# OPPO-Mente-Lab/X2I

Hardware: AMD Instinct MI355X
Metric: images/sec, FLUX-schnell 1024x1024 4-step (projector + denoise loop), whole job (higher is better)
Workload: dtype bf16; 1 GPU; BASELINE configs[1]: qwen3b conditioning (C=37,H=2048,S_txt=512) -> projector -> shuttle-3/FLUX-schnell DiT 1024x1024, 4 steps; batch_per_gpu=4, global_batch=4, parallelism=batch-sharded x1, graph=True

## Files before the change

### x2i_amd/csrc/c_api.hip

```cpp
#include <stdarg.h>
#include <stdio.h>

#include "x2i_common.h"
#include "x2i_kernels.h"

static thread_local char g_err[512] = "";

int x2i_set_error(int code, const char* fmt, ...) {
  va_list ap;
  va_start(ap, fmt);
  vsnprintf(g_err, sizeof(g_err), fmt, ap);
  va_end(ap);
  return code;
}

int x2i_check_launch(const char* what) {
  hipError_t e = hipGetLastError();
  if (e != hipSuccess) return x2i_set_error(X2I_ERR_HIP, "%s: launch failed: %s", what, hipGetErrorString(e));
  return X2I_OK;
}

#include <stdlib.h>
#include <string.h>

// ... 7 lines not shown
  return v && *v ? atoi(v) : dflt;
}
X2IOptions make_options() {
  X2IOptions o;
  o.gemm_tile = env_int("X2I_GEMM_TILE", 0);
  o.gemm_min256 = env_int("X2I_GEMM_MIN256", 128);
  o.gemm_gm = env_int("X2I_GEMM_GM", 0);
  o.gemm_split_tail = env_int("X2I_GEMM_NOSPLIT", 0) ? 0 : 1;
  o.gemm_w4 = env_int("X2I_GEMM_W4", 1);
  o.gemm_persist = env_int("X2I_GEMM_PERSIST", 1);
  o.gemm_fp8_persist = env_int("X2I_GEMM_FP8_PERSIST", 1);
  o.gemm_fx = env_int("X2I_GEMM_FX", 2);
  o.gemm_fx_nk = env_int("X2I_GEMM_FX_NK", 96);
  o.gemm_streamk = env_int("X2I_GEMM_STREAMK", 1);
  o.gemm_pair = env_int("X2I_GEMM_PAIR", 1);
  o.train_rows_wg = env_int("X2I_TRAIN_ROWS_WG", 1);
  o.attn_bwd_overlap = env_int("X2I_ATTN_BWD_OVERLAP", 1);
  o.conv256 = env_int("X2I_CONV256", 1);
  o.conv_w4 = env_int("X2I_CONV_W4", 1);
  o.conv_korder = env_int("X2I_CONV_KORDER", 1);
  o.attn_variant = env_int("X2I_ATTN_VARIANT", 0);
  o.attn_w16 = env_int("X2I_ATTN_W16", 1);
  o.attn_streamk = env_int("X2I_ATTN_STREAMK", 1);
  o.conv5_variant = env_int("X2I_CONV5_VARIANT", 0);
  o.fp8 = env_int("X2I_FP8", 0);
  o.last_gemm_tile = -1;
  o.attn_ablate = env_int("X2I_ATTN_ABLATE", 0);
  return o;
}
std::mutex g_smem_mu;
std::set<std::pair<const void*, int>> g_smem_done;
}

X2IOptions& x2i_options() {
  static X2IOptions o = make_options();
  return o;
}

int x2i_ensure_dynamic_smem(const void* kernel, int bytes) {
  int dev = 0;
  hipGetDevice(&dev);
// ... 28 lines not shown
                        need, (long long)a->workspace_bytes);
    return false;
  }
  *flags = (unsigned*)a->workspace;
  *slabs = (float*)((char*)a->workspace + 4096);
  return true;
}

extern "C" {

int x2i_abi_version(void) { return X2I_ABI_VERSION; }

static long long* opt_slot(X2IOptions& o, const char* name, int** as_int) {
  *as_int = nullptr;
#define X2I_OPT_INT(N_) if (!strcmp(name, #N_)) { *as_int = &o.N_; return nullptr; }
  X2I_OPT_INT(gemm_tile) X2I_OPT_INT(gemm_gm) X2I_OPT_INT(gemm_split_tail) X2I_OPT_INT(gemm_w4) X2I_OPT_INT(gemm_persist) X2I_OPT_INT(gemm_fp8_persist) X2I_OPT_INT(gemm_fx) X2I_OPT_INT(gemm_fx_nk) X2I_OPT_INT(gemm_streamk) X2I_OPT_INT(gemm_pair) X2I_OPT_INT(train_rows_wg) X2I_OPT_INT(attn_bwd_overlap) X2I_OPT_INT(attn_streamk) X2I_OPT_INT(conv256) X2I_OPT_INT(conv_w4) X2I_OPT_INT(conv_korder) X2I_OPT_INT(attn_variant) X2I_OPT_INT(attn_w16) X2I_OPT_INT(conv5_variant) X2I_OPT_INT(fp8) X2I_OPT_INT(last_gemm_tile)
#ifdef X2I_ABLATION
  X2I_OPT_INT(attn_ablate)
#endif
#undef X2I_OPT_INT
  if (!strcmp(name, "gemm_min256")) return &o.gemm_min256;
  return nullptr;
}

int x2i_set_option(const char* name, int64_t value) {
  if (!name) return x2i_set_error(X2I_ERR_ARG, "set_option: null name");
  int* ip;
  long long* lp = opt_slot(x2i_options(), name, &ip);
  if (ip) *ip = (int)value;
  else if (lp) *lp = (long long)value;
  else return x2i_set_error(X2I_ERR_ARG, "set_option: unknown option '%s'", name);
// ... 361 lines not shown
```

### x2i_amd/csrc/gemm.hip

```cpp
#include "gemm_device.h"

using namespace x2i_gemm;

namespace {

__global__ void gemm_naive_kernel(GemmP p, int batch) {
  const int n = blockIdx.x * blockDim.x + threadIdx.x;
  const long long mz = (long long)blockIdx.z * gridDim.y + blockIdx.y;
  const int z = (int)(mz / p.M), m = (int)(mz % p.M);
  if (n >= p.N || z >= batch) return;
  const bf16_t* a = p.A + (long long)z * p.a_bs + (long long)m * p.lda;
  const bf16_t* w = p.W + (long long)(z / p.wdiv) * p.w_bs + (long long)n * p.ldw;
  float acc = 0.f;
  for (int k = 0; k < p.K; ++k) acc = fmaf(bf16_to_f32(a[k]), bf16_to_f32(w[k]), acc);
  float v = acc + (p.bias ? bf16_to_f32(p.bias[(long long)(z / p.wdiv) * p.bias_gs + n]) : 0.f) + (p.bias2 ? p.bias2[(long long)z * p.bias2_bs + n] : 0.f);
  v = apply_act(v, p.act);
  if (p.res) {
    const float g = p.gate ? p.gate[(long long)z * p.gate_bs + n] : 1.f;
    v = fmaf(g, v, bf16_to_f32(p.res[(long long)z * p.r_bs + (long long)m * p.ldr + n]));
  }
  const long long coff = (long long)z * p.c_bs + (long long)m * p.ldc + n;
  if (p.out_f32) ((float*)p.C)[coff] = v;
  else ((bf16_t*)p.C)[coff] = f32_to_bf16(v);
  if (p.C2) p.C2[coff] = f32_to_bf16(apply_act(v, p.act2));
// ... 21 lines not shown
}

static void fill_gemm_p(const x2i_gemm_args* a, const x2i_qkv_desc* qd, GemmP& p) {
  p.A = (const bf16_t*)a->A; p.a_bs = a->a_batch_stride; p.lda = a->lda;
  p.W = (const bf16_t*)a->W; p.ldw = a->ldw; p.w_bs = a->w_batch_stride;
  p.wdiv = a->w_group > 0 ? a->w_group : 1; p.bias_gs = a->w_group > 0 ? a->N : 0;
  p.bias = (const bf16_t*)a->bias;
  p.C = a->C; p.c_bs = a->c_batch_stride; p.ldc = a->ldc;
  p.C2 = (bf16_t*)a->C2; p.act2 = a->act2;
  p.gate = a->gate; p.gate_bs = a->gate_batch_stride;
  p.res = (const bf16_t*)a->res; p.r_bs = a->res_batch_stride; p.ldr = a->ldr;
  p.bias2 = a->bias2; p.bias2_bs = a->bias2_batch_stride;
  p.M = a->M; p.N = a->N; p.K = a->K; p.act = a->act; p.out_f32 = a->out_f32;
  p.cH = p.cW = p.cCin = p.cOW = p.cKW = p.cStride = p.cPad = p.cUp = p.cPadW = p.cRowPitch = p.cKorder = 0; p.cMom = nullptr; p.cMomBlocks = 0;
  p.gm = 4;
  p.q_on = 0; p.q_H = p.q_Spad = p.q_tok_off = p.q_rpb = p.q_row0 = p.q_vperm = 0; p.q_eps = 0.f; p.q_qs = 1.f;
  p.q_nq = p.q_nk = nullptr; p.q_cos = p.q_sin = nullptr; p.q_Q = p.q_K = p.q_VT = nullptr;
  p.f_sa = p.f_sw = nullptr; p.f_sa_bs = 0; p.f_alpha = p.f_oinv = 1.f; p.f_out8 = 0;
  p.nbatch = 1; p.sk_on = 0; p.sk_slabs = nullptr; p.sk_flags = nullptr; p.fx_v0 = 0;
  if (qd) {
    p.q_on = 1; p.q_H = qd->H; p.q_Spad = qd->Spad; p.q_tok_off = qd->tok_off; p.q_rpb = qd->rows_per_sample; p.q_eps = qd->eps; p.q_qs = qd->q_scale == 0.f ? 1.f : qd->q_scale;
    p.q_nq = (const bf16_t*)qd->norm_q; p.q_nk = (const bf16_t*)qd->norm_k; p.q_cos = qd->cos; p.q_sin = qd->sin;
    p.q_Q = (bf16_t*)qd->Q; p.q_K = (bf16_t*)qd->K; p.q_VT = (bf16_t*)qd->VT; p.q_vperm = qd->vt_perm ? 1 : 0;
    p.ldc = a->N; p.c_bs = 0;
  }
}

static int pick_gm(int tn, int K) {
  const X2IOptions& opt = x2i_options();
  if (opt.gemm_gm > 0) return opt.gemm_gm;
  if (tn <= 16) return K >= 8192 ? 1 : 4;
  if (tn <= 64) return 6;
  return 2;
}

static bool persistent_ok(const x2i_gemm_args* a, const x2i_qkv_desc* qd) {
  const X2IOptions& opt = x2i_options();
  const bool res = a->res != nullptr;
  const bool fast = (a->K % BK == 0) && (a->lda % 8 == 0) && (a->ldw % 8 == 0) && (((uintptr_t)a->A & 15) == 0) && (((uintptr_t)a->W & 15) == 0) &&
                    ((a->a_batch_stride & 7) == 0) && ((long long)a->M * a->lda * 2 < 0x7f000000LL) && ((long long)a->N * a->ldw * 2 < 0x7f000000LL);
// ... 75 lines not shown
    if (rc) return rc;
    pp.p[0].fx_v0 = v0;
    for (int i = 0; i < 2; ++i) pp.p[i].sk_slabs = sk_slabs, pp.p[i].sk_flags = sk_flags;
    hipLaunchKernelGGL(kfx, dim3((unsigned)cus), dim3(256), SMEM2P_BYTES, stream, pp);
    opt.last_gemm_tile = 3256;
    return x2i_check_launch("gemm_pair (fx)");
  }
  if (rc) return rc;
  rc = x2i_ensure_dynamic_smem((const void*)kern, SMEM2P_BYTES);
  if (rc) return rc;
  const bool sk = streamk_for(a0, tiles, a0->K / BK, cus, &sk_slabs, &sk_flags, &rc);
  if (rc) return rc;
  pp.p[0].sk_on = sk ? 1 : 0; pp.p[0].sk_slabs = sk_slabs; pp.p[0].sk_flags = sk_flags;
  hipLaunchKernelGGL(kern, dim3((unsigned)(tiles < cus ? tiles : cus)), dim3(256), SMEM2P_BYTES, stream, pp);
  opt.last_gemm_tile = 2256;
  return x2i_check_launch("gemm_pair");
}

constexpr int MOM_SLABS = 64;
__device__ __forceinline__ f32x4_t mom_block_sum(const float* __restrict__ src, int r0, int r1, int n2, f32x4_t* red) {
  const int lanes = n2 >> 2, groups = 256 / lanes;
  const int l = threadIdx.x % lanes, g = threadIdx.x / lanes;
  f32x4_t a0 = {0.f, 0.f, 0.f, 0.f}, a1 = a0, a2 = a0, a3 = a0;
  if (g < groups) {
    const float* p = src + 4 * l;
    int rb = r0 + g;
    for (; rb + 3 * groups < r1; rb += 4 * groups) {
      a0 += *(const f32x4_t*)(p + (long long)rb * n2);
      a1 += *(const f32x4_t*)(p + (long long)(rb + groups) * n2);
      a2 += *(const f32x4_t*)(p + (long long)(rb + 2 * groups) * n2);
// ... 92 lines not shown
      if (rc) return rc;
    }
  }
  return x2i_check_launch("conv");
}

static int launch_gemm_impl(const x2i_gemm_args* a, const x2i_conv_desc* cd, const x2i_qkv_desc* qd, hipStream_t stream) {
  if (!a || !a->A || !a->W || (!a->C && !qd)) return x2i_set_error(X2I_ERR_ARG, "gemm: null pointer");
  const bool conv = cd != nullptr;
  if (a->M <= 0 || a->N <= 0 || a->K <= 0 || a->batch <= 0) return x2i_set_error(X2I_ERR_SHAPE, "gemm: bad shape M=%d N=%d K=%d batch=%d", a->M, a->N, a->K, a->batch);
  if (a->gate && !a->res) return x2i_set_error(X2I_ERR_ARG, "gemm: gate without residual");
  if (a->w_group < 0 || (a->w_group > 0 && (!a->w_batch_stride || qd || a->C2 || a->out_f32)))
    return x2i_set_error(X2I_ERR_ARG, "gemm: w_group=%d needs w_batch_stride != 0 and goes with the plain bf16 outputs only (no fused QKV / C2 / f32 output)", a->w_group);
  GemmP p;
  fill_gemm_p(a, qd, p);
  if (conv) {
    if (a->gate) return x2i_set_error(X2I_ERR_ARG, "conv: a gated residual is not part of the convolution epilogues (residual: plain add)");
    if (cd->Cin % 64 || cd->H <= 0 || cd->W <= 0 || cd->KH <= 0 || cd->KW <= 0 || cd->stride <= 0)
      return x2i_set_error(X2I_ERR_SHAPE, "conv: Cin must be a multiple of 64 (Cin=%d)", cd->Cin);
    if (cd->up < 0 || cd->up > 2) return x2i_set_error(X2I_ERR_ARG, "conv: up must be 0, 1 (x2 along H and W) or 2 (x2 along H only), got %d", cd->up);
    const int up_h = cd->up ? 1 : 0, up_w = cd->up == 1 ? 1 : 0, up = up_h | (up_w << 1);
    const int pad_w = cd->pad_w_p1 <= 0 ? cd->pad : cd->pad_w_p1 - 1;
    if (cd->KH * cd->KW > 32) return x2i_set_error(X2I_ERR_SHAPE, "conv: at most 32 filter taps (KH=%d KW=%d)", cd->KH, cd->KW);
    int OH = ((cd->H << up_h) + 2 * cd->pad - cd->KH) / cd->stride + 1;
    if (cd->out_h) {
      if (cd->out_h < 0 || (cd->out_h - 1) * cd->stride - cd->pad >= (cd->H << up_h)) return x2i_set_error(X2I_ERR_SHAPE, "conv: out_h=%d lies outside the input (H=%d pad=%d)", cd->out_h, cd->H, cd->pad);
      OH = cd->out_h;
    }
    int OW = ((cd->W << up_w) + 2 * pad_w - cd->KW) / cd->stride + 1;
    if (cd->out_w) {
// ... 128 lines not shown
    int tm_main = tm_all;
    if (!sk && force == 0 && !conv && full_rounds >= 1 && rem > 0 && (rem <= 96 || (rem <= 128 && full_rounds >= 8)) && opt.gemm_split_tail) {
      const long long tm_fit = (full_rounds * 256) / per_row;
      if (tm_fit >= 1 && tm_fit < tm_all) tm_main = (int)tm_fit;
    }
    GemmP pm = p;
    pm.gm = pick_gm(tn, a->K);
    pm.M = (tm_main < tm_all) ? tm_main * BM2 : a->M;
    pm.tilesM = tm_main; pm.tilesN = tn;
    pm.cMomBlocks = tm_main * 2;
    if (kernp) {
      rc = x2i_ensure_dynamic_smem((const void*)kernp, SMEM2P_BYTES);
      if (rc) return rc;
      pm.nbatch = a->batch;
      pm.sk_on = sk ? 1 : 0; pm.sk_slabs = sk_slabs; pm.sk_flags = sk_flags;
      const long long tiles = (long long)pm.tilesM * pm.tilesN * a->batch;
      hipLaunchKernelGGL(kernp, dim3((unsigned)(tiles < cus ? tiles : cus)), dim3(256), SMEM2P_BYTES, stream, pm);
    } else {
      hipLaunchKernelGGL(kern2, dim3(pm.tilesM * pm.tilesN, a->batch), dim3(threads2), SMEM2_BYTES, stream, pm);
    }
    opt.last_gemm_tile = 256 + (tm_main < tm_all ? 1000 : 0);
    if (tm_main < tm_all) {
      rc = x2i_ensure_dynamic_smem((const void*)kern, 4 * TILE_BYTES);
      if (rc) return rc;
      GemmP pt = p;
      const long long r0 = (long long)tm_main * BM2;
      pt.A = p.A + r0 * p.lda;
      pt.C = p.out_f32 ? (void*)((float*)p.C + r0 * p.ldc) : (void*)((bf16_t*)p.C + r0 * p.ldc);
      if (p.C2) pt.C2 = p.C2 + r0 * p.ldc;
      if (p.res) pt.res = p.res + r0 * p.ldr;
// ... 77 lines not shown
    return x2i_set_error(X2I_ERR_ALIGN, "gemm_fp8: N, ldc and c_batch_stride must be multiples of %d, C 16-byte aligned", nal + 1);
  if (out8 && (res || a->gate)) return x2i_set_error(X2I_ERR_ARG, "gemm_fp8: e4m3 output has no residual form");
  kern_t kern = pick_gemm256_fp8(a->act, res, out8);
  if (!kern) return x2i_set_error(X2I_ERR_ARG, "gemm_fp8: epilogue (act=%d%s%s) is not instantiated", a->act, res ? ", residual" : "", out8 ? ", e4m3 out" : "");
  GemmP p;
  p.A = (const bf16_t*)a->A; p.a_bs = a->a_batch_stride; p.lda = a->lda;
  p.W = (const bf16_t*)a->W; p.ldw = a->ldw; p.w_bs = 0; p.wdiv = 1; p.bias_gs = 0;
  p.bias = (const bf16_t*)a->bias;
  p.C = a->C; p.c_bs = a->c_batch_stride; p.ldc = a->ldc;
  p.C2 = nullptr; p.act2 = 0;
  p.gate = a->gate; p.gate_bs = a->gate_batch_stride;
  p.res = (const bf16_t*)a->res; p.r_bs = a->res_batch_stride; p.ldr = a->ldr;
  p.bias2 = a->bias2; p.bias2_bs = a->bias2_batch_stride;
  p.M = a->M; p.N = a->N; p.K = a->K; p.act = a->act; p.out_f32 = 0;
  p.cH = p.cW = p.cCin = p.cOW = p.cKW = p.cStride = p.cPad = p.cUp = p.cPadW = p.cRowPitch = p.cKorder = 0; p.cMom = nullptr; p.cMomBlocks = 0;
  p.q_on = 0; p.q_H = p.q_Spad = p.q_tok_off = p.q_rpb = p.q_row0 = p.q_vperm = 0; p.q_eps = 0.f; p.q_qs = 1.f;
  p.q_nq = p.q_nk = nullptr; p.q_cos = p.q_sin = nullptr; p.q_Q = p.q_K = p.q_VT = nullptr;
  if (qd) {
    p.q_on = 1; p.q_H = qd->H; p.q_Spad = qd->Spad; p.q_tok_off = qd->tok_off; p.q_rpb = qd->rows_per_sample; p.q_eps = qd->eps; p.q_qs = qd->q_scale == 0.f ? 1.f : qd->q_scale;
    p.q_nq = (const bf16_t*)qd->norm_q; p.q_nk = (const bf16_t*)qd->norm_k; p.q_cos = qd->cos; p.q_sin = qd->sin;
    p.q_Q = (bf16_t*)qd->Q; p.q_K = (bf16_t*)qd->K; p.q_VT = (bf16_t*)qd->VT; p.q_vperm = qd->vt_perm ? 1 : 0;
    p.ldc = a->N; p.c_bs = 0;
  }
  p.f_sa = f->a_scale; p.f_sa_bs = f->a_scale_batch_stride; p.f_sw = f->w_scale; p.f_alpha = f->alpha; p.f_oinv = f->out_inv_scale;
  p.f_out8 = out8 ? 1 : 0;
  p.nbatch = 1; p.sk_on = 0; p.sk_slabs = nullptr; p.sk_flags = nullptr; p.fx_v0 = 0;
#ifdef X2I_ABLATION
  p.act2 = a->act2;
#endif
  const int tm = (a->M + BM2 - 1) / BM2, tn = (a->N + BN2 - 1) / BN2;
  p.tilesM = tm; p.tilesN = tn;
// ... 36 lines not shown
```

### x2i_amd/csrc/gemm256p.hip

```cpp
#include <type_traits>
#include "gemm_device.h"
#include "gemm256p_epi.h"
#include "gemm256w_loop.inc"
#include "gemm256f8_loop.inc"

namespace x2i_gemm {
namespace {

__device__ __forceinline__ void epilogue_fx_slice(const GemmP& p, int z, int m_wave, int n_wave, int lane, char* stage, int slab0, int P, int j,
                                                  int tid) {
  typedef unsigned int u32x4 __attribute__((ext_vector_type(4)));
  typedef unsigned int u32x2 __attribute__((ext_vector_type(2)));
  const int mlane = lane & 15, ng = lane >> 4;
  const int srow = lane >> 3, sch = lane & 7;
  const float* b2 = p.bias2 ? p.bias2 + (long long)z * p.bias2_bs : nullptr;
#ifdef X2I_ABLATION
  if (p.act2 >= 80) b2 = nullptr;
#endif
  const float* gz = p.gate ? p.gate + (long long)z * p.gate_bs : nullptr;
  __amdgpu_buffer_rsrc_t r_rsrc = __builtin_amdgcn_make_buffer_rsrc((void*)(p.res + (long long)z * p.r_bs), 0, (uint32_t)(((long long)(p.M - 1) * p.ldr + p.N) * 2), 0x00020000);
  const uint32_t c_bytes = (uint32_t)(((long long)(p.M - 1) * p.ldc + p.N) * 2);
  __amdgpu_buffer_rsrc_t c_rsrc = __builtin_amdgcn_make_buffer_rsrc((void*)((bf16_t*)p.C + (long long)z * p.c_bs), 0, c_bytes, 0x00020000);
  const float* sbase = p.sk_slabs + (long long)slab0 * (SK_SLAB_BYTES / 4) + tid * 4;
  for (int q = j; q < 8; q += P) {
// ... 323 lines not shown
};

template <bool PAIR> using GemmArg = std::conditional_t<PAIR, GemmP2, GemmP>;
__device__ __forceinline__ const GemmP& prob(const GemmP& a, int) { return a; }
__device__ __forceinline__ const GemmP& first(const GemmP& a) { return a; }
__device__ __forceinline__ const GemmP& first(const GemmP2& a) { return a.p[0]; }
__device__ __forceinline__ const GemmP& second(const GemmP& a) { return a; }
__device__ __forceinline__ const GemmP& second(const GemmP2& a) { return a.p[1]; }
__device__ __forceinline__ GemmP prob(const GemmP2& a, int sel) {
  const GemmP &x = a.p[0], &y = a.p[1];
  GemmP q;
#define X2I_F(f) q.f = sel ? y.f : x.f;
  X2I_F(A) X2I_F(a_bs) X2I_F(lda) X2I_F(W) X2I_F(ldw) X2I_F(w_bs) X2I_F(bias) X2I_F(C) X2I_F(c_bs) X2I_F(ldc) X2I_F(C2) X2I_F(act2)
  X2I_F(gate) X2I_F(gate_bs) X2I_F(res) X2I_F(r_bs) X2I_F(ldr) X2I_F(bias2) X2I_F(bias2_bs) X2I_F(M) X2I_F(N) X2I_F(K) X2I_F(act)
  X2I_F(out_f32) X2I_F(tilesM) X2I_F(tilesN) X2I_F(cH) X2I_F(cW) X2I_F(cCin) X2I_F(cOW) X2I_F(cKW) X2I_F(cStride) X2I_F(cPad) X2I_F(cUp) X2I_F(cPadW) X2I_F(cRowPitch) X2I_F(cKorder) X2I_F(cMom) X2I_F(cMomBlocks)
  X2I_F(q_on) X2I_F(q_H) X2I_F(q_Spad) X2I_F(q_tok_off) X2I_F(q_rpb) X2I_F(q_row0) X2I_F(q_vperm) X2I_F(gm) X2I_F(q_eps) X2I_F(q_qs) X2I_F(q_nq) X2I_F(q_nk)
  X2I_F(q_cos) X2I_F(q_sin) X2I_F(q_Q) X2I_F(q_K) X2I_F(q_VT) X2I_F(f_sa) X2I_F(f_sa_bs) X2I_F(f_sw) X2I_F(f_alpha) X2I_F(f_oinv) X2I_F(f_out8)
  X2I_F(nbatch) X2I_F(sk_on) X2I_F(sk_slabs) X2I_F(sk_flags) X2I_F(fx_v0)
#undef X2I_F
  return q;
}

template <int ACT, bool RES, bool HASC2, bool QKV = false, bool PAIR = false, bool F8 = false, bool OUT8 = false, bool FX = false>
__global__ __launch_bounds__(256) void gemm256p_kernel(GemmArg<PAIR> pp) {
  constexpr int ES = F8 ? 1 : 2;
  constexpr int KT = F8 ? 128 : BK;
  extern __shared__ __attribute__((aligned(16))) char smem[];
  const GemmP& p = first(pp);
  const int tid = threadIdx.x;
  const int lane = tid & 63;
  const int wave = __builtin_amdgcn_readfirstlane(tid >> 6);
// ... 11 lines not shown
    const int v = vb - sel * TT0;
    z = v / T;
    int bid = v - z * T;
    const int qq = T >> 3, r = T & 7, xcd = bid & 7, idx = bid >> 3;
    bid = (xcd < r ? xcd * (qq + 1) : r * (qq + 1) + (xcd - r) * qq) + idx;
    const int GM = q.gm;
    const int per_group = GM * q.tilesN;
    const int group = bid / per_group;
    const int first_m = group * GM;
    const int gsize = min(q.tilesM - first_m, GM);
    m0 = (first_m + (bid % per_group) % gsize) * BM2;
    n0 = ((bid % per_group) / gsize) * BN2;
  };
  const int khl = lane >> 5, r8 = (lane >> 2) & 7, cphys = lane & 3;
  const int kby = khl * 64 + ((cphys ^ (3 * (wave & 1))) << 4);
  auto offsets = [&](int sel, int z, int m0, int n0, uint32_t (&va)[8], uint32_t (&vw)[8]) {
    const GemmP& q = prob(pp, sel);
#ifdef X2I_ABLATION
    if (p.act2 == 75) m0 = 0, n0 = 0;
    if (p.act2 == 76) m0 &= 1023, n0 &= 2047;
#endif
    const long long zoff = (long long)z * q.a_bs;
#pragma unroll
    for (int jj = 0; jj < 8; ++jj) {
      const int row = (jj * 4 + wave) * 8 + r8;
      va[jj] = (m0 + row < q.M) ? (uint32_t)((zoff + (long long)(m0 + row) * q.lda) * ES + kby) : 0x80000000u;
      vw[jj] = (n0 + row < q.N) ? (uint32_t)(((long long)(n0 + row) * q.ldw) * ES + kby) : 0x80000000u;
    }
  };
  auto uni = [](auto v) { return (decltype(v))__builtin_amdgcn_readfirstlane((int)v); };
  auto mk_rsrc = [&](const void* ptr, uint32_t bytes) {
    const unsigned long long a = (unsigned long long)(uintptr_t)ptr;
    const unsigned long long au = ((unsigned long long)(unsigned)uni((int)(a >> 32)) << 32) | (unsigned)uni((int)(a & 0xffffffffu));
    return __builtin_amdgcn_make_buffer_rsrc((void*)(uintptr_t)au, 0, (uint32_t)uni((int)bytes), 0x00020000);
  };
  auto a_rsrc_of = [&](int sel) {
    const GemmP& q = prob(pp, sel);
    return mk_rsrc(q.A, (uint32_t)(((long long)(q.nbatch - 1) * q.a_bs + (long long)(q.M - 1) * q.lda + q.K) * ES));
  };
  auto w_rsrc_of = [&](int sel) {
    const GemmP& q = prob(pp, sel);
    return mk_rsrc(q.W, (uint32_t)(((long long)(q.N - 1) * q.ldw + q.K) * ES));
  };
  int fx_sel = 0, fx_Tp = 0, fx_nbz = 0, fx_kind = 0, fx_cnt = 0, fx_t0 = 0, fx_tstep = 1, fx_k0 = 0, fx_len = 0, fx_npre = 0, fx_modeB = 0, fx_slab_base = 0, fx_part = 0;
  const int fx_x = w & 7;
  if constexpr (FX) {
    const int wi = w >> 3, Gx = G >> 3;
    const int v0 = p.fx_v0;
    fx_sel = PAIR ? min(max(wi - v0 + 1, 0), 1) : 0;
    const GemmP& q = prob(pp, fx_sel);
    const int li = wi - fx_sel * v0, v = fx_sel ? Gx - v0 : v0;
    fx_Tp = q.tilesM * q.tilesN;
    fx_nbz = q.nbatch;
    fx_slab_base = fx_sel * (first(pp).tilesM * first(pp).tilesN);
    const int Tx = fx_Tp >> 3;
    if (v < 2 * Tx) {
      fx_modeB = 1;
// ... 124 lines not shown
    if (tid == 0) {
      for (int q = 0; q < P; ++q) fx_spin(fx_flag(buf, uslab0 + 8 * q), (unsigned)utag, 8u, 0xffffffu);
      __builtin_amdgcn_fence(__ATOMIC_ACQUIRE, "agent");
    }
    __syncthreads();
    epilogue_fx_slice(prob(pp, usel), uz, um0 + wm * 128, un0 + wn * 128, lane, stage, uslab0 + 256 * buf, P, fx_part, tid);
    __syncthreads();
    if (tid == 0)
      for (int q = 0; q < P; ++q) __hip_atomic_fetch_add(fx_flag(buf, uslab0 + 8 * q), 1u, __ATOMIC_RELAXED, __HIP_MEMORY_SCOPE_AGENT);
  };
  int pend_valid = 0, pend_sel = 0, pend_z = 0, pend_m0 = 0, pend_n0 = 0, pend_slab0 = 0, pend_tag = 0;
  Unit cur = unit(0);
  int sel, z, m0, n0;
  tile_of(cur.vb, sel, z, m0, n0);
  uint32_t va[8], vw[8], na[8], nw[8];
  offsets(sel, z, m0, n0, va, vw);
  __amdgpu_buffer_rsrc_t a_rsrc = a_rsrc_of(sel), w_rsrc = w_rsrc_of(sel);
  bf16x8_t fr[F8 ? 1 : 32];
  uint32_t s_koff, s_it, s_so;
  int k0b = cur.k0 * 128;
  if constexpr (F8) {
    asm volatile(X2I_GEMM256F8_PRO
                 : [koff] "=&s"(s_koff)
                 : X2I_GEMM256W_OPS_VOFF(va, vw), [dma] "s"(dma), [ra] "s"(a_rsrc), [rw] "s"(w_rsrc), [k0b] "s"(k0b)
                 : "memory", "scc", "m0");
  } else {
    asm volatile(X2I_GEMM256P_PRO
                 : X2I_GEMM256P_OPS_FRAG0_OUT(fr), [koff] "=&s"(s_koff)
                 : X2I_GEMM256W_OPS_VOFF(va, vw), [la] "v"(la), [lw] "v"(lw), [dma] "s"(dma), [ra] "s"(a_rsrc), [rw] "s"(w_rsrc), [k0b] "s"(k0b)
                 : "memory", "scc", "m0");
  }
  for (int ui = 0;; ++ui) {
    const Unit nxt = unit(ui + 1);
    const bool has_next = nxt.vb >= 0;
    int nsel = PAIR ? min(max(nxt.vb - TT0 + 1, 0), 1) : 0, nz = 0, nm0 = 0, nn0 = 0;
    if constexpr (PAIR) a_rsrc = a_rsrc_of(sel), w_rsrc = w_rsrc_of(sel);
    const __amdgpu_buffer_rsrc_t na_rsrc = PAIR ? a_rsrc_of(nsel) : a_rsrc, nw_rsrc = PAIR ? w_rsrc_of(nsel) : w_rsrc;
    if (has_next) {
      tile_of(nxt.vb, nsel, nz, nm0, nn0);
      offsets(nsel, nz, nm0, nn0, na, nw);
    } else {
#pragma unroll
      for (int jj = 0; jj < 8; ++jj) na[jj] = nw[jj] = 0x80000000u;
    }
    const int nk0b = nxt.k0 * 128, len = cur.len;
    f32x4_t acc[2][4][2][4];
    const int fromp = FX ? 0 : min(cur.k0, 1);
    if (fromp) {
      unsigned* flag = p.sk_flags + cur.slab;
      if (tid == 0) {
        int spins = 0;
        while (__hip_atomic_load(flag, __ATOMIC_RELAXED, __HIP_MEMORY_SCOPE_AGENT) != (unsigned)cur.k0) {
          __builtin_amdgcn_s_sleep(32);
          if (++spins > (1 << 22)) {
            __hip_atomic_store(p.sk_flags + SK_ERR_SLOT, 1u, __ATOMIC_RELAXED, __HIP_MEMORY_SCOPE_AGENT);
            break;
          }
        }
        __builtin_amdgcn_fence(__ATOMIC_ACQUIRE, "agent");
      }
      __syncthreads();
    }
    __amdgpu_buffer_rsrc_t s_rsrc = slab_rsrc(cur.slab < 0 ? 0 : cur.slab);
    asm volatile(X2I_GEMM256P_LOAD_PARTIAL
                 : X2I_GEMM256P_OPS_ACC_OUT(acc), [so] "=&s"(s_so)
                 : [vo] "v"(slab_vo), [rs] "s"(s_rsrc), [fromp] "s"(fromp)
                 : "memory", "scc");
    const int zs = 1 - fromp;
    Deq<F8> dq;
    deq_load<F8>(prob(pp, sel), z, m0 + wm * 128, n0 + wn * 128, lane, dq);
#ifdef X2I_ABLATION
    unsigned long long* tdbg = (p.act2 >= 79 && tid == 0 && w < 16) ? (unsigned long long*)p.bias2 + w * 64 : nullptr;
    if (tdbg && ui < 31) tdbg[2 * ui] = __builtin_amdgcn_s_memrealtime();
#endif
    if constexpr (F8) {
      asm volatile(X2I_GEMM256F8_MAIN
                   : X2I_GEMM256P_OPS_ACC_IO(acc), [la] "+v"(la), [lw] "+v"(lw), [dma] "+s"(dma), [koff] "=&s"(s_koff), [it] "=&s"(s_it)
                   : X2I_GEMM256W_OPS_VOFF(va, vw), X2I_GEMM256P_OPS_NEXT(na, nw), [ra] "s"(a_rsrc), [rw] "s"(w_rsrc), [nra] "s"(na_rsrc),
                     [nrw] "s"(nw_rsrc), [nk] "s"(len), [k0b] "s"(k0b), [nk0b] "s"(nk0b), [zs] "s"(zs)
                   : "memory", "scc", "m0", X2I_GEMM256F8_FRAG_CLOBBERS);
    } else {
      asm volatile(X2I_GEMM256P_MAIN
                   : X2I_GEMM256P_OPS_ACC_IO(acc), X2I_GEMM256P_OPS_FRAG0_IO(fr), X2I_GEMM256P_OPS_FRAG1(fr), [la] "+v"(la), [lw] "+v"(lw),
                     [dma] "+s"(dma), [koff] "=&s"(s_koff), [it] "=&s"(s_it)
                   : X2I_GEMM256W_OPS_VOFF(va, vw), X2I_GEMM256P_OPS_NEXT(na, nw), [ra] "s"(a_rsrc), [rw] "s"(w_rsrc), [nra] "s"(na_rsrc),
                     [nrw] "s"(nw_rsrc), [nk] "s"(len),
                     [k0b] "s"(k0b), [nk0b] "s"(nk0b), [zs] "s"(zs)
                   : "memory", "scc", "m0");
    }
#ifdef X2I_ABLATION
    if (tdbg && ui < 31) tdbg[2 * ui + 1] = __builtin_amdgcn_s_memrealtime();
#endif
    auto spin_until = [&](unsigned* flag, unsigned want) {
      int spins = 0;
      while (__hip_atomic_load(flag, __ATOMIC_RELAXED, __HIP_MEMORY_SCOPE_AGENT) != want) {
        __builtin_amdgcn_s_sleep(32);
        if (++spins > (1 << 22)) {
          __hip_atomic_store(p.sk_flags + SK_ERR_SLOT, 1u, __ATOMIC_RELAXED, __HIP_MEMORY_SCOPE_AGENT);
          break;
        }
      }
    };
// ... 39 lines not shown
    } else if (cur.k0 + cur.len < nk) {
      __amdgpu_buffer_rsrc_t s_rsrc = slab_rsrc(cur.slab);
      asm volatile(X2I_GEMM256P_STORE_PARTIAL
                   : [so] "=&s"(s_so)
                   : X2I_GEMM256P_OPS_ACC_IN(acc), [vo] "v"(slab_vo), [rs] "s"(s_rsrc)
                   : "memory", "scc");
      __syncthreads();
      if (tid == 0) __hip_atomic_store(p.sk_flags + cur.slab, (unsigned)(cur.k0 + cur.len), __ATOMIC_RELAXED, __HIP_MEMORY_SCOPE_AGENT);
    } else {
      if (cur.k0 > 0 && tid == 0) __hip_atomic_store(p.sk_flags + cur.slab, 0u, __ATOMIC_RELAXED, __HIP_MEMORY_SCOPE_AGENT);
#ifdef X2I_ABLATION
      if (p.act2 == 77 || p.act2 == 79) {
        asm volatile("" ::X2I_GEMM256P_OPS_ACC_IN(acc));
      } else
#endif
      if constexpr (QKV) epilogue_qkv_chunked<F8>(prob(pp, sel), acc, z, m0 + wm * 128, n0 + wn * 128, lane, stage, dq);
      else if constexpr (OUT8) {
        if (p.f_oinv == 1.f) epilogue_chunked_pipe_e4m3<ACT, true>(prob(pp, sel), acc, z, m0 + wm * 128, n0 + wn * 128, lane, stage, dq);
        else epilogue_chunked_pipe_e4m3<ACT, false>(prob(pp, sel), acc, z, m0 + wm * 128, n0 + wn * 128, lane, stage, dq);
      } else epilogue_chunked_pipe<ACT, HASC2, RES, F8>(prob(pp, sel), acc, z, m0 + wm * 128, n0 + wn * 128, lane, stage, dq);
    }
    if (!has_next) break;
    cur = nxt; sel = nsel; z = nz; m0 = nm0; n0 = nn0; k0b = nk0b;

#pragma unroll
    for (int jj = 0; jj < 8; ++jj) va[jj] = na[jj], vw[jj] = nw[jj];
  }
  if constexpr (FX) {
    if (pend_valid) {
      const int last = (n_units - 1) & 1;
      fx_slice_of(pend_sel, pend_z, pend_m0, pend_n0, pend_slab0, pend_tag, last);
      if (n_units >= 2) fx_reclaim(last ^ 1);
      fx_reclaim(last);
    }
  }
  asm volatile(X2I_GEMM256P_DRAIN ::: "memory");
}

}

kern_t pick_gemm256p_qkv() { return gemm256p_kernel<X2I_ACT_NONE, false, false, true>; }
// ... 43 lines not shown
```

### x2i_amd/csrc/gemm256p_epi.h

```cpp
#pragma once
#include <type_traits>
#include "gemm_device.h"

namespace x2i_gemm {
namespace {

constexpr int P_STAGE_OFF = 2 * TILE2_BYTES;
constexpr int P_STAGE_WAVE = 8192;

template <bool F8> struct Deq {};
template <> struct Deq<true> {
  float sw[8][4];
  float sr[4][2];
};
template <bool F8>
__device__ __forceinline__ void deq_load(const GemmP& p, int z, int m_wave, int n_wave, int lane, Deq<F8>& d) {
  if constexpr (F8) {
    const int ng = lane >> 4, mlane = lane & 15;
    static_for<8>([&](auto jc) {
      constexpr int j = decltype(jc)::value;
      const int n = n_wave + j * 16 + ng * 4;
      f32x4_t v = {1.f, 1.f, 1.f, 1.f};
      if (p.f_sw) v = *(const f32x4_t*)(p.f_sw + (n < p.N ? n : 0));
#pragma unroll
// ... 339 lines not shown
        }
      }
      __builtin_amdgcn_raw_buffer_store_b128(d[j], pass == 0 ? c_rsrc : c2_rsrc, vo, soff, 0);
    });
  });
  if constexpr (CONV) {
    if (p.cMom) {
      static_for<8>([&](auto jc) {
        constexpr int j = decltype(jc)::value;
        mom_flush(p, mom_s[j], mom_q[j], z, m_wave >> 7, n_wave + j * 16 + ng * 4, lane);
      });
    }
  }
}

}
}
```

### x2i_amd/csrc/gemm_device.h

```cpp
#pragma once
#include "x2i_common.h"
#include "x2i_kernels.h"
#include <type_traits>

namespace x2i_gemm {

constexpr int BM = 128, BN = 128, BK = 64;
constexpr int TILE_BYTES = BM * BK * 2;

struct GemmP {
  const bf16_t* A; long long a_bs; int lda;
  const bf16_t* W; int ldw; long long w_bs;
  int wdiv, bias_gs;
  const bf16_t* bias;
  void* C; long long c_bs; int ldc;
  bf16_t* C2; int act2;
  const float* gate; long long gate_bs;
  const bf16_t* res; long long r_bs; int ldr;
  const float* bias2; long long bias2_bs;
  int M, N, K;
  int act, out_f32;
  int tilesM, tilesN;
  int cH, cW, cCin, cOW, cKW, cStride, cPad, cUp;
  int cPadW;
  int cRowPitch;
  int cKorder;
  float* cMom; int cMomBlocks;
  int q_on, q_H, q_Spad, q_tok_off, q_rpb, q_row0, q_vperm;
  int gm;
  float q_eps, q_qs;
  const bf16_t *q_nq, *q_nk;
  const float *q_cos, *q_sin;
  bf16_t *q_Q, *q_K, *q_VT;
  const float* f_sa; long long f_sa_bs;
  const float* f_sw;
  float f_alpha, f_oinv;
  int f_out8;
  int nbatch, sk_on;
  float* sk_slabs;
  unsigned* sk_flags;
  int fx_v0;
};
struct GemmP2 { GemmP p[2]; };
// ... 498 lines not shown
```

### x2i_amd/csrc/x2i_common.h

```cpp
#pragma once
#include <hip/hip_runtime.h>
#include <stdint.h>

typedef uint16_t bf16_t;
typedef __attribute__((ext_vector_type(8))) short bf16x8_t;
typedef __attribute__((ext_vector_type(4))) short bf16x4_t;
typedef __attribute__((ext_vector_type(4))) float f32x4_t;
typedef __attribute__((ext_vector_type(16))) float f32x16_t;

#define X2I_OK 0
#define X2I_ERR_ARG (-1)
#define X2I_ERR_SHAPE (-2)
#define X2I_ERR_ALIGN (-3)
#define X2I_ERR_HIP (-4)
#define X2I_ERR_STATE (-5)

int x2i_set_error(int code, const char* fmt, ...);
int x2i_check_launch(const char* what);

struct X2IOptions {
  int gemm_tile;
  long long gemm_min256;
  int gemm_gm;
  int gemm_split_tail;
  int gemm_w4;
  int attn_bwd_overlap;
  int train_rows_wg;
  int gemm_pair;
  int gemm_streamk;
  int gemm_fx_nk;
  int gemm_fx;
  int gemm_fp8_persist;
  int gemm_persist;
  int conv256;
  int conv_w4;
  int conv_korder;
  int attn_variant;
  int attn_w16;
  int attn_streamk;
  int conv5_variant;
  int fp8;
  int last_gemm_tile;
  int attn_ablate;
};
X2IOptions& x2i_options();
int x2i_ensure_dynamic_smem(const void* kernel, int bytes);
int x2i_num_cus();
struct x2i_gemm_args;
bool x2i_streamk_workspace(const x2i_gemm_args* a, float** slabs, unsigned** flags, int* rc);
long long x2i_conv_moments_scratch(int M, int N, int batch);
int x2i_conv_moments_reduce(float* scratch, float* moments, int batch, int blocks, int N, int accumulate, hipStream_t stream);
int x2i_gemm_sk_slabs();
int x2i_gemm_sk_max_tiles();
long long x2i_gemm_sk_slab_bytes();

__device__ __forceinline__ int x2i_vt_pos(int t, int perm) {
  return perm ? ((t & ~31) | (((t >> 2) & 3) << 3) | (((t >> 4) & 1) << 2) | (t & 3)) : t;
// ... 92 lines not shown
```

Before: 4.518 images/s.

## Swap GEMM operands for V tiles in fused QKV to write V-transpose directly

For fused QKV projection tiles that fall in the V section, the persistent 256 GEMM kernel swaps the A and W operands so the accumulator comes out already transposed. A new epilogue then writes V^T rows with coalesced 128-bit buffer stores through a swizzled LDS stage. This targets the scattered transposed stores of the old V^T epilogue. The cost is extra per-tile offset and resource recomputation, plus more scalar uniformity casts in the main loop.

```diff
diff --git a/x2i_amd/csrc/c_api.hip b/x2i_amd/csrc/c_api.hip
--- a/x2i_amd/csrc/c_api.hip
+++ b/x2i_amd/csrc/c_api.hip
@@ -45,6 +45,7 @@
   o.gemm_fx_nk = env_int("X2I_GEMM_FX_NK", 96);
   o.gemm_streamk = env_int("X2I_GEMM_STREAMK", 1);
   o.gemm_pair = env_int("X2I_GEMM_PAIR", 1);
+  o.qkv_vswap = env_int("X2I_QKV_VSWAP", 1);
   o.train_rows_wg = env_int("X2I_TRAIN_ROWS_WG", 1);
   o.attn_bwd_overlap = env_int("X2I_ATTN_BWD_OVERLAP", 1);
   o.conv256 = env_int("X2I_CONV256", 1);
@@ -56,6 +57,7 @@
   o.conv5_variant = env_int("X2I_CONV5_VARIANT", 0);
   o.fp8 = env_int("X2I_FP8", 0);
   o.last_gemm_tile = -1;
+  o.last_qkv_vswap = 0;
   o.attn_ablate = env_int("X2I_ATTN_ABLATE", 0);
   return o;
 }
@@ -114,7 +116,7 @@
 static long long* opt_slot(X2IOptions& o, const char* name, int** as_int) {
   *as_int = nullptr;
 #define X2I_OPT_INT(N_) if (!strcmp(name, #N_)) { *as_int = &o.N_; return nullptr; }
-  X2I_OPT_INT(gemm_tile) X2I_OPT_INT(gemm_gm) X2I_OPT_INT(gemm_split_tail) X2I_OPT_INT(gemm_w4) X2I_OPT_INT(gemm_persist) X2I_OPT_INT(gemm_fp8_persist) X2I_OPT_INT(gemm_fx) X2I_OPT_INT(gemm_fx_nk) X2I_OPT_INT(gemm_streamk) X2I_OPT_INT(gemm_pair) X2I_OPT_INT(train_rows_wg) X2I_OPT_INT(attn_bwd_overlap) X2I_OPT_INT(attn_streamk) X2I_OPT_INT(conv256) X2I_OPT_INT(conv_w4) X2I_OPT_INT(conv_korder) X2I_OPT_INT(attn_variant) X2I_OPT_INT(attn_w16) X2I_OPT_INT(conv5_variant) X2I_OPT_INT(fp8) X2I_OPT_INT(last_gemm_tile)
+  X2I_OPT_INT(gemm_tile) X2I_OPT_INT(gemm_gm) X2I_OPT_INT(gemm_split_tail) X2I_OPT_INT(gemm_w4) X2I_OPT_INT(gemm_persist) X2I_OPT_INT(gemm_fp8_persist) X2I_OPT_INT(gemm_fx) X2I_OPT_INT(gemm_fx_nk) X2I_OPT_INT(gemm_streamk) X2I_OPT_INT(gemm_pair) X2I_OPT_INT(qkv_vswap) X2I_OPT_INT(train_rows_wg) X2I_OPT_INT(attn_bwd_overlap) X2I_OPT_INT(attn_streamk) X2I_OPT_INT(conv256) X2I_OPT_INT(conv_w4) X2I_OPT_INT(conv_korder) X2I_OPT_INT(attn_variant) X2I_OPT_INT(attn_w16) X2I_OPT_INT(conv5_variant) X2I_OPT_INT(fp8) X2I_OPT_INT(last_gemm_tile) X2I_OPT_INT(last_qkv_vswap)
 #ifdef X2I_ABLATION
   X2I_OPT_INT(attn_ablate)
 #endif
diff --git a/x2i_amd/csrc/gemm.hip b/x2i_amd/csrc/gemm.hip
--- a/x2i_amd/csrc/gemm.hip
+++ b/x2i_amd/csrc/gemm.hip
@@ -59,7 +59,7 @@
   p.M = a->M; p.N = a->N; p.K = a->K; p.act = a->act; p.out_f32 = a->out_f32;
   p.cH = p.cW = p.cCin = p.cOW = p.cKW = p.cStride = p.cPad = p.cUp = p.cPadW = p.cRowPitch = p.cKorder = 0; p.cMom = nullptr; p.cMomBlocks = 0;
   p.gm = 4;
-  p.q_on = 0; p.q_H = p.q_Spad = p.q_tok_off = p.q_rpb = p.q_row0 = p.q_vperm = 0; p.q_eps = 0.f; p.q_qs = 1.f;
+  p.q_on = 0; p.q_H = p.q_Spad = p.q_tok_off = p.q_rpb = p.q_row0 = p.q_vperm = p.q_vswap = 0; p.q_eps = 0.f; p.q_qs = 1.f;
   p.q_nq = p.q_nk = nullptr; p.q_cos = p.q_sin = nullptr; p.q_Q = p.q_K = p.q_VT = nullptr;
   p.f_sa = p.f_sw = nullptr; p.f_sa_bs = 0; p.f_alpha = p.f_oinv = 1.f; p.f_out8 = 0;
   p.nbatch = 1; p.sk_on = 0; p.sk_slabs = nullptr; p.sk_flags = nullptr; p.fx_v0 = 0;
@@ -69,6 +69,13 @@
     p.q_Q = (bf16_t*)qd->Q; p.q_K = (bf16_t*)qd->K; p.q_VT = (bf16_t*)qd->VT; p.q_vperm = qd->vt_perm ? 1 : 0;
     p.ldc = a->N; p.c_bs = 0;
   }
+}
+
+static int qkv_vswap_ok(const GemmP& p) {
+  if (!p.q_on || !x2i_options().qkv_vswap) return 0;
+  if (((p.q_tok_off | p.q_Spad | p.M) & 7) || ((p.q_rpb | p.q_row0) & 127) || p.q_Spad >= (1 << 22)) return 0;
+  if (p.q_vperm && ((p.M | p.q_tok_off) & 31)) return 0;
+  return 1;
 }
 
 static int pick_gm(int tn, int K) {
@@ -174,6 +181,7 @@
   pp.p[0].sk_on = sk ? 1 : 0; pp.p[0].sk_slabs = sk_slabs; pp.p[0].sk_flags = sk_flags;
   hipLaunchKernelGGL(kern, dim3((unsigned)(tiles < cus ? tiles : cus)), dim3(256), SMEM2P_BYTES, stream, pp);
   opt.last_gemm_tile = 2256;
+  if (q0) opt.last_qkv_vswap = 0;
   return x2i_check_launch("gemm_pair");
 }
 
@@ -296,6 +304,7 @@
     return x2i_set_error(X2I_ERR_ARG, "gemm: w_group=%d needs w_batch_stride != 0 and goes with the plain bf16 outputs only (no fused QKV / C2 / f32 output)", a->w_group);
   GemmP p;
   fill_gemm_p(a, qd, p);
+  if (qd) x2i_options().last_qkv_vswap = 0;
   if (conv) {
     if (a->gate) return x2i_set_error(X2I_ERR_ARG, "conv: a gated residual is not part of the convolution epilogues (residual: plain add)");
     if (cd->Cin % 64 || cd->H <= 0 || cd->W <= 0 || cd->KH <= 0 || cd->KW <= 0 || cd->stride <= 0)
@@ -454,6 +463,8 @@
       if (rc) return rc;
       pm.nbatch = a->batch;
       pm.sk_on = sk ? 1 : 0; pm.sk_slabs = sk_slabs; pm.sk_flags = sk_flags;
+      pm.q_vswap = qkv_vswap_ok(pm);
+      if (qd) opt.last_qkv_vswap = pm.q_vswap;
       const long long tiles = (long long)pm.tilesM * pm.tilesN * a->batch;
       hipLaunchKernelGGL(kernp, dim3((unsigned)(tiles < cus ? tiles : cus)), dim3(256), SMEM2P_BYTES, stream, pm);
     } else {
@@ -561,7 +572,7 @@
   p.bias2 = a->bias2; p.bias2_bs = a->bias2_batch_stride;
   p.M = a->M; p.N = a->N; p.K = a->K; p.act = a->act; p.out_f32 = 0;
   p.cH = p.cW = p.cCin = p.cOW = p.cKW = p.cStride = p.cPad = p.cUp = p.cPadW = p.cRowPitch = p.cKorder = 0; p.cMom = nullptr; p.cMomBlocks = 0;
-  p.q_on = 0; p.q_H = p.q_Spad = p.q_tok_off = p.q_rpb = p.q_row0 = p.q_vperm = 0; p.q_eps = 0.f; p.q_qs = 1.f;
+  p.q_on = 0; p.q_H = p.q_Spad = p.q_tok_off = p.q_rpb = p.q_row0 = p.q_vperm = p.q_vswap = 0; p.q_eps = 0.f; p.q_qs = 1.f;
   p.q_nq = p.q_nk = nullptr; p.q_cos = p.q_sin = nullptr; p.q_Q = p.q_K = p.q_VT = nullptr;
   if (qd) {
     p.q_on = 1; p.q_H = qd->H; p.q_Spad = qd->Spad; p.q_tok_off = qd->tok_off; p.q_rpb = qd->rows_per_sample; p.q_eps = qd->eps; p.q_qs = qd->q_scale == 0.f ? 1.f : qd->q_scale;
diff --git a/x2i_amd/csrc/gemm256p.hip b/x2i_amd/csrc/gemm256p.hip
--- a/x2i_amd/csrc/gemm256p.hip
+++ b/x2i_amd/csrc/gemm256p.hip
@@ -361,7 +361,7 @@
   X2I_F(A) X2I_F(a_bs) X2I_F(lda) X2I_F(W) X2I_F(ldw) X2I_F(w_bs) X2I_F(bias) X2I_F(C) X2I_F(c_bs) X2I_F(ldc) X2I_F(C2) X2I_F(act2)
   X2I_F(gate) X2I_F(gate_bs) X2I_F(res) X2I_F(r_bs) X2I_F(ldr) X2I_F(bias2) X2I_F(bias2_bs) X2I_F(M) X2I_F(N) X2I_F(K) X2I_F(act)
   X2I_F(out_f32) X2I_F(tilesM) X2I_F(tilesN) X2I_F(cH) X2I_F(cW) X2I_F(cCin) X2I_F(cOW) X2I_F(cKW) X2I_F(cStride) X2I_F(cPad) X2I_F(cUp) X2I_F(cPadW) X2I_F(cRowPitch) X2I_F(cKorder) X2I_F(cMom) X2I_F(cMomBlocks)
-  X2I_F(q_on) X2I_F(q_H) X2I_F(q_Spad) X2I_F(q_tok_off) X2I_F(q_rpb) X2I_F(q_row0) X2I_F(q_vperm) X2I_F(gm) X2I_F(q_eps) X2I_F(q_qs) X2I_F(q_nq) X2I_F(q_nk)
+  X2I_F(q_on) X2I_F(q_H) X2I_F(q_Spad) X2I_F(q_tok_off) X2I_F(q_rpb) X2I_F(q_row0) X2I_F(q_vperm) X2I_F(q_vswap) X2I_F(gm) X2I_F(q_eps) X2I_F(q_qs) X2I_F(q_nq) X2I_F(q_nk)
   X2I_F(q_cos) X2I_F(q_sin) X2I_F(q_Q) X2I_F(q_K) X2I_F(q_VT) X2I_F(f_sa) X2I_F(f_sa_bs) X2I_F(f_sw) X2I_F(f_alpha) X2I_F(f_oinv) X2I_F(f_out8)
   X2I_F(nbatch) X2I_F(sk_on) X2I_F(sk_slabs) X2I_F(sk_flags) X2I_F(fx_v0)
 #undef X2I_F
@@ -403,18 +403,36 @@
   };
   const int khl = lane >> 5, r8 = (lane >> 2) & 7, cphys = lane & 3;
   const int kby = khl * 64 + ((cphys ^ (3 * (wave & 1))) << 4);
-  auto offsets = [&](int sel, int z, int m0, int n0, uint32_t (&va)[8], uint32_t (&vw)[8]) {
+  constexpr bool VSWAP = QKV && !F8 && !PAIR;
+  auto swap_of = [&](int sel, int n0) -> int {
+    if constexpr (!VSWAP) return 0;
+    const GemmP& q = prob(pp, sel);
+    return __builtin_amdgcn_readfirstlane(q.q_vswap * min(max(n0 - 2 * q.q_H * 128 + 1, 0), 1));
+  };
+  auto offsets = [&](int sel, int z, int m0, int n0, int sw, uint32_t (&va)[8], uint32_t (&vw)[8]) {
     const GemmP& q = prob(pp, sel);
 #ifdef X2I_ABLATION
     if (p.act2 == 75) m0 = 0, n0 = 0;
     if (p.act2 == 76) m0 &= 1023, n0 &= 2047;
 #endif
     const long long zoff = (long long)z * q.a_bs;
-#pragma unroll
-    for (int jj = 0; jj < 8; ++jj) {
-      const int row = (jj * 4 + wave) * 8 + r8;
-      va[jj] = (m0 + row < q.M) ? (uint32_t)((zoff + (long long)(m0 + row) * q.lda) * ES + kby) : 0x80000000u;
-      vw[jj] = (n0 + row < q.N) ? (uint32_t)(((long long)(n0 + row) * q.ldw) * ES + kby) : 0x80000000u;
+    if constexpr (VSWAP) {
+      const int x = sw ? 1 : 0;
+      const int ra0 = x ? n0 : m0, rw0 = x ? m0 : n0, lima = x ? q.N : q.M, limw = x ? q.M : q.N, pa = x ? q.ldw : q.lda, pw = x ? q.lda : q.ldw;
+      const long long za = x ? 0 : zoff, zw = x ? zoff : 0;
+#pragma unroll
+      for (int jj = 0; jj < 8; ++jj) {
+        const int row = (jj * 4 + wave) * 8 + r8;
+        va[jj] = (ra0 + row < lima) ? (uint32_t)((za + (long long)(ra0 + row) * pa) * ES + kby) : 0x80000000u;
+        vw[jj] = (rw0 + row < limw) ? (uint32_t)((zw + (long long)(rw0 + row) * pw) * ES + kby) : 0x80000000u;
+      }
+    } else {
+#pragma unroll
+      for (int jj = 0; jj < 8; ++jj) {
+        const int row = (jj * 4 + wave) * 8 + r8;
+        va[jj] = (m0 + row < q.M) ? (uint32_t)((zoff + (long long)(m0 + row) * q.lda) * ES + kby) : 0x80000000u;
+        vw[jj] = (n0 + row < q.N) ? (uint32_t)(((long long)(n0 + row) * q.ldw) * ES + kby) : 0x80000000u;
+      }
     }
   };
   auto uni = [](auto v) { return (decltype(v))__builtin_amdgcn_readfirstlane((int)v); };
@@ -423,13 +441,17 @@
     const unsigned long long au = ((unsigned long long)(unsigned)uni((int)(a >> 32)) << 32) | (unsigned)uni((int)(a & 0xffffffffu));
     return __builtin_amdgcn_make_buffer_rsrc((void*)(uintptr_t)au, 0, (uint32_t)uni((int)bytes), 0x00020000);
   };
-  auto a_rsrc_of = [&](int sel) {
+  auto a_rsrc_of = [&](int sel, int sw = 0) {
     const GemmP& q = prob(pp, sel);
-    return mk_rsrc(q.A, (uint32_t)(((long long)(q.nbatch - 1) * q.a_bs + (long long)(q.M - 1) * q.lda + q.K) * ES));
-  };
-  auto w_rsrc_of = [&](int sel) {
+    const uint32_t ab = (uint32_t)(((long long)(q.nbatch - 1) * q.a_bs + (long long)(q.M - 1) * q.lda + q.K) * ES);
+    if constexpr (VSWAP) return mk_rsrc(sw ? (const void*)q.W : (const void*)q.A, sw ? (uint32_t)(((long long)(q.N - 1) * q.ldw + q.K) * ES) : ab);
+    else return mk_rsrc(q.A, ab);
+  };
+  auto w_rsrc_of = [&](int sel, int sw = 0) {
     const GemmP& q = prob(pp, sel);
-    return mk_rsrc(q.W, (uint32_t)(((long long)(q.N - 1) * q.ldw + q.K) * ES));
+    const uint32_t wb = (uint32_t)(((long long)(q.N - 1) * q.ldw + q.K) * ES);
+    if constexpr (VSWAP) return mk_rsrc(sw ? (const void*)q.A : (const void*)q.W, sw ? (uint32_t)(((long long)(q.nbatch - 1) * q.a_bs + (long long)(q.M - 1) * q.lda + q.K) * ES) : wb);
+    else return mk_rsrc(q.W, wb);
   };
   int fx_sel = 0, fx_Tp = 0, fx_nbz = 0, fx_kind = 0, fx_cnt = 0, fx_t0 = 0, fx_tstep = 1, fx_k0 = 0, fx_len = 0, fx_npre = 0, fx_modeB = 0, fx_slab_base = 0, fx_part = 0;
   const int fx_x = w & 7;
@@ -584,8 +606,9 @@
   int sel, z, m0, n0;
   tile_of(cur.vb, sel, z, m0, n0);
   uint32_t va[8], vw[8], na[8], nw[8];
-  offsets(sel, z, m0, n0, va, vw);
-  __amdgpu_buffer_rsrc_t a_rsrc = a_rsrc_of(sel), w_rsrc = w_rsrc_of(sel);
+  int sw = swap_of(sel, n0);
+  offsets(sel, z, m0, n0, sw, va, vw);
+  __amdgpu_buffer_rsrc_t a_rsrc = a_rsrc_of(sel, sw), w_rsrc = w_rsrc_of(sel, sw);
   bf16x8_t fr[F8 ? 1 : 32];
   uint32_t s_koff, s_it, s_so;
   int k0b = cur.k0 * 128;
@@ -604,11 +627,15 @@
     const Unit nxt = unit(ui + 1);
     const bool has_next = nxt.vb >= 0;
     int nsel = PAIR ? min(max(nxt.vb - TT0 + 1, 0), 1) : 0, nz = 0, nm0 = 0, nn0 = 0;
-    if constexpr (PAIR) a_rsrc = a_rsrc_of(sel), w_rsrc = w_rsrc_of(sel);
-    const __amdgpu_buffer_rsrc_t na_rsrc = PAIR ? a_rsrc_of(nsel) : a_rsrc, nw_rsrc = PAIR ? w_rsrc_of(nsel) : w_rsrc;
+    if constexpr (VSWAP) {
+      if (has_next) tile_of(nxt.vb, nsel, nz, nm0, nn0);
+    }
+    const int nsw = swap_of(nsel, nn0);
+    if constexpr (PAIR || VSWAP) a_rsrc = a_rsrc_of(sel, sw), w_rsrc = w_rsrc_of(sel, sw);
+    const __amdgpu_buffer_rsrc_t na_rsrc = (PAIR || VSWAP) ? a_rsrc_of(nsel, nsw) : a_rsrc, nw_rsrc = (PAIR || VSWAP) ? w_rsrc_of(nsel, nsw) : w_rsrc;
     if (has_next) {
-      tile_of(nxt.vb, nsel, nz, nm0, nn0);
-      offsets(nsel, nz, nm0, nn0, na, nw);
+      if constexpr (!VSWAP) tile_of(nxt.vb, nsel, nz, nm0, nn0);
+      offsets(nsel, nz, nm0, nn0, nsw, na, nw);
     } else {
 #pragma unroll
       for (int jj = 0; jj < 8; ++jj) na[jj] = nw[jj] = 0x80000000u;
@@ -637,6 +664,8 @@
                  : [vo] "v"(slab_vo), [rs] "s"(s_rsrc), [fromp] "s"(fromp)
                  : "memory", "scc");
     const int zs = 1 - fromp;
+    auto sc = [&](int v) { if constexpr (VSWAP) return uni(v); else return v; };
+    if constexpr (VSWAP) dma = (uint32_t)uni((int)dma);
     Deq<F8> dq;
     deq_load<F8>(prob(pp, sel), z, m0 + wm * 128, n0 + wn * 128, lane, dq);
 #ifdef X2I_ABLATION
@@ -654,8 +683,8 @@
                    : X2I_GEMM256P_OPS_ACC_IO(acc), X2I_GEMM256P_OPS_FRAG0_IO(fr), X2I_GEMM256P_OPS_FRAG1(fr), [la] "+v"(la), [lw] "+v"(lw),
                      [dma] "+s"(dma), [koff] "=&s"(s_koff), [it] "=&s"(s_it)
                    : X2I_GEMM256W_OPS_VOFF(va, vw), X2I_GEMM256P_OPS_NEXT(na, nw), [ra] "s"(a_rsrc), [rw] "s"(w_rsrc), [nra] "s"(na_rsrc),
-                     [nrw] "s"(nw_rsrc), [nk] "s"(len),
-                     [k0b] "s"(k0b), [nk0b] "s"(nk0b), [zs] "s"(zs)
+                     [nrw] "s"(nw_rsrc), [nk] "s"(sc(len)),
+                     [k0b] "s"(sc(k0b)), [nk0b] "s"(sc(nk0b)), [zs] "s"(sc(zs))
                    : "memory", "scc", "m0");
     }
 #ifdef X2I_ABLATION
@@ -725,17 +754,23 @@
         asm volatile("" ::X2I_GEMM256P_OPS_ACC_IN(acc));
       } else
 #endif
-      if constexpr (QKV) epilogue_qkv_chunked<F8>(prob(pp, sel), acc, z, m0 + wm * 128, n0 + wn * 128, lane, stage, dq);
-      else if constexpr (OUT8) {
+      if constexpr (QKV) {
+        if (VSWAP && sw) epilogue_vt_swapped_pipe(prob(pp, sel), acc, z, m0 + wn * 128, n0 + wm * 128, lane, stage);
+        else epilogue_qkv_chunked<F8>(prob(pp, sel), acc, z, m0 + wm * 128, n0 + wn * 128, lane, stage, dq);
+      } else if constexpr (OUT8) {
         if (p.f_oinv == 1.f) epilogue_chunked_pipe_e4m3<ACT, true>(prob(pp, sel), acc, z, m0 + wm * 128, n0 + wn * 128, lane, stage, dq);
         else epilogue_chunked_pipe_e4m3<ACT, false>(prob(pp, sel), acc, z, m0 + wm * 128, n0 + wn * 128, lane, stage, dq);
       } else epilogue_chunked_pipe<ACT, HASC2, RES, F8>(prob(pp, sel), acc, z, m0 + wm * 128, n0 + wn * 128, lane, stage, dq);
     }
     if (!has_next) break;
-    cur = nxt; sel = nsel; z = nz; m0 = nm0; n0 = nn0; k0b = nk0b;
-
-#pragma unroll
-    for (int jj = 0; jj < 8; ++jj) va[jj] = na[jj], vw[jj] = nw[jj];
+    cur = nxt; sel = nsel; z = nz; m0 = nm0; n0 = nn0; k0b = nk0b; sw = nsw;
+
+    if constexpr (VSWAP) {
+      offsets(sel, z, m0, n0, sw, va, vw);
+    } else {
+#pragma unroll
+      for (int jj = 0; jj < 8; ++jj) va[jj] = na[jj], vw[jj] = nw[jj];
+    }
   }
   if constexpr (FX) {
     if (pend_valid) {
diff --git a/x2i_amd/csrc/gemm256p_epi.h b/x2i_amd/csrc/gemm256p_epi.h
--- a/x2i_amd/csrc/gemm256p_epi.h
+++ b/x2i_amd/csrc/gemm256p_epi.h
@@ -377,5 +377,70 @@
   }
 }
 
-}
-}
+__device__ __forceinline__ void epilogue_vt_swapped_pipe(const GemmP& p, f32x4_t (&acc)[2][4][2][4], int z, int t_wave, int d_wave, int lane, char* stage) {
+  typedef unsigned int u32x4 __attribute__((ext_vector_type(4)));
+  asm volatile("" : "+v"(lane));
+  const int mlane = lane & 15, ng = lane >> 4;
+  const int srow = lane >> 3, sch = lane & 7;
+  const int head = (d_wave - 2 * p.q_H * 128) >> 7;
+  const TokMap tmap = tok_map(p, z, t_wave);
+  const int b = tmap.b0, st0 = tmap.tok_off + tmap.r0;
+  float bv[4][2];
+#pragma unroll
+  for (int c = 0; c < 4; ++c)
+#pragma unroll
+    for (int i = 0; i < 2; ++i) bv[c][i] = p.bias ? bf16_to_f32(p.bias[d_wave + c * 32 + i * 16 + mlane]) : 0.f;
+  const unsigned long long va = (unsigned long long)(uintptr_t)(p.q_VT + ((long long)(b * p.q_H + head) * 128) * p.q_Spad + st0);
+  const unsigned long long vu = ((unsigned long long)(unsigned)__builtin_amdgcn_readfirstlane((int)(va >> 32)) << 32) | (unsigned)__builtin_amdgcn_readfirstlane((int)(va & 0xffffffffu));
+  __amdgpu_buffer_rsrc_t v_rsrc = __builtin_amdgcn_make_buffer_rsrc((void*)(uintptr_t)vu, 0, (uint32_t)((127 * p.q_Spad + 128) * 2), 0x00020000);
+  auto voff = [&](int h, int it) {
+    const int row = it * 8 + srow;
+    const int pc = h * 64 + ((sch ^ ((row >> 1) & 7)) << 3);
+    return (t_wave + pc < p.M) ? (uint32_t)((row * p.q_Spad + pc) * 2) : 0x80000000u;
+  };
+  const int vperm = p.q_vperm;
+  asm volatile("" ::: "memory");
+  auto stage_a = [&](auto qc, auto jc, int which) {
+    constexpr int q = decltype(qc)::value;
+    constexpr int j = decltype(jc)::value;
+    constexpr int h = q >> 2, c = q & 3;
+    char* buf = stage + which * 4096;
+    const int grp = vperm ? (((j >> 1) << 2) | ng) : ((j << 1) | (ng >> 1));
+    const int half = vperm ? (j & 1) : (ng & 1);
+    static_for<2>([&](auto ic) {
+      constexpr int i = decltype(ic)::value;
+      float v[4];
+#pragma unroll
+      for (int r = 0; r < 4; ++r) {
+        float t;
+        const float a = acc[h][c][i][j][r];
+        asm volatile("v_accvgpr_read_b32 %0, %1" : "=v"(t) : "a"(a));
+        v[r] = t + bv[c][i];
+      }
+      const int row = i * 16 + mlane;
+      *(uint2*)(buf + row * 128 + ((grp ^ ((row >> 1) & 7)) << 4) + (half << 3)) = make_uint2(pack_bf16x2(v[0], v[1]), pack_bf16x2(v[2], v[3]));
+    });
+  };
+  u32x4 d[4];
+  static_for<4>([&](auto jc) { stage_a(std::integral_constant<int, 0>{}, jc, 0); });
+  static_for<8>([&](auto qc) {
+    constexpr int q = decltype(qc)::value;
+    constexpr int h = q >> 2, c = q & 3;
+    char* buf = stage + (q & 1) * 4096;
+    __builtin_amdgcn_sched_barrier(0);
+    asm volatile("s_waitcnt lgkmcnt(0)" ::: "memory");
+#pragma unroll
+    for (int it = 0; it < 4; ++it) d[it] = *(const u32x4*)(buf + it * 1024 + lane * 16);
+    const uint32_t soff = (uint32_t)(c * 32 * p.q_Spad * 2);
+    static_for<4>([&](auto jc) {
+      constexpr int j = decltype(jc)::value;
+      __builtin_amdgcn_sched_barrier(0);
+      if constexpr (q + 1 < 8) stage_a(std::integral_constant<int, q + 1>{}, jc, (q + 1) & 1);
+      __builtin_amdgcn_sched_barrier(0);
+      __builtin_amdgcn_raw_buffer_store_b128(d[j], v_rsrc, voff(h, j), soff, 0);
+    });
+  });
+}
+
+}
+}
diff --git a/x2i_amd/csrc/gemm_device.h b/x2i_amd/csrc/gemm_device.h
--- a/x2i_amd/csrc/gemm_device.h
+++ b/x2i_amd/csrc/gemm_device.h
@@ -27,6 +27,7 @@
   int cKorder;
   float* cMom; int cMomBlocks;
   int q_on, q_H, q_Spad, q_tok_off, q_rpb, q_row0, q_vperm;
+  int q_vswap;
   int gm;
   float q_eps, q_qs;
   const bf16_t *q_nq, *q_nk;
diff --git a/x2i_amd/csrc/x2i_common.h b/x2i_amd/csrc/x2i_common.h
--- a/x2i_amd/csrc/x2i_common.h
+++ b/x2i_amd/csrc/x2i_common.h
@@ -27,6 +27,7 @@
   int attn_bwd_overlap;
   int train_rows_wg;
   int gemm_pair;
+  int qkv_vswap;
   int gemm_streamk;
   int gemm_fx_nk;
   int gemm_fx;
@@ -41,6 +42,7 @@
   int conv5_variant;
   int fp8;
   int last_gemm_tile;
+  int last_qkv_vswap;
   int attn_ablate;
 };
 X2IOptions& x2i_options();
```

Result: no change. 4.532 images/s, median of 6 (+0.3%).
